# qurAI-amsterdam/SuperResolution_aniso_MRI

Hardware: AMD Instinct MI355X
Metric: training slices/sec (ae_combined, 160x160, latent=128) (higher is better)
Workload: dtype f32; 1 GPU; ACDC synthetic 12x(3x1x160x160) triplets, ae_combined latent=128 depth=32 scales=2, MSE synthesis loss (BASELINE configs[1]); global_batch_triplets=12, parallelism=dp1, init=reference Initializer, seed 892372, random weights, launch=captured HIP graph replay

## Files before the change

superresolution_aniso_mri_amd/csrc/aesr_kernels.h:

```cpp
#pragma once
#include "aesr_common.h"

struct IgemmArgs {
    const float* in; const float* wpk; const float* bias; const float* ysave; float* out;
    int N, H, W, Cin, CinP, Cout, CoutP, Ho, Wo, pad;
    int TI, TH, TW, tiles_y, tiles_x, nitems, dbg;
    int unused_;
    int ksplit;
    float* dbgbuf;
    int act, mask_act;
    float slope;
};
int aesr_launch_conv_igemm(const IgemmArgs& a, int KS, int NB, int MBW, hipStream_t st);
int aesr_launch_conv_ksplit_fixup(const float* partial, const float* bias, const float* ysave, float* out, size_t nelem, int Cout,
                                  int ksplit, int act, int mask_act, float slope, hipStream_t st);
int aesr_launch_pack_weights(const float* w, float* p, int Cout, int Cin, int KS, int KinP, int NoutP, int TN, int transpose, hipStream_t st);

struct WinoArgs {
    const float* in; const float* upk; const float* bias; const float* ysave; float* out;
    int N, H, W, Cin, CinP, Cout, CoutP;
    int TI, THt, TWt;
    int regs_y, regs_x, nitems;
    unsigned m_ncot, m_regs_x, m_regs_y;
    int act, mask_act;
    float slope;
    float* dbgbuf;
    int flags;
    int in_up2;
    int out_sum2;
    int bpi, nblk;
    unsigned m_bpi;
    int nw, rowP, imgP, patch_fl, sw_a, sw_m, sw_b;
    int xcd_map;
    double plan_cost;
    int nfull, tail_k;
    int ksplit, kchunks, split_bytes;
    unsigned m_ksplit;
    float* ws;
    size_t ws_floats;
    const float* post_scale; const float* post_shift;
    int post_pool;
};
int aesr_launch_conv_wino(const WinoArgs& a, hipStream_t st);
bool aesr_wino_res_ok(const WinoArgs& a);
int aesr_launch_conv_wino_res(const WinoArgs& a, hipStream_t st);
int aesr_wino_ring_mode();
bool aesr_wino_ring_takes(const WinoArgs& a);
int aesr_launch_conv_wino_ring(const WinoArgs& a, hipStream_t st);
size_t aesr_wino_ring_workspace_floats(const WinoArgs& a);
unsigned aesr_wino_ring_timeouts();
size_t aesr_wino_lds_bytes(int patch_pixels);

#define PACK_MAX_JOBS 32
struct PackJob { const float* w; float* p; int Cout, Cin, KS, KinP, NoutP, TN, transpose, block0; };
struct PackTable { int njobs, nblocks; PackJob job[PACK_MAX_JOBS]; };
int aesr_launch_pack_many(const PackTable& t, hipStream_t st);
enum { PREP_PACK = 0, PREP_WINO_PACK = 1, PREP_STEM_FOLD = 2, PREP_COUT1_FLIP = 3 };
struct PrepJob { const float* w; const float* aux0; const float* aux1; float* out; int kind, Cout, Cin, KS, KinP, NoutP, TN, transpose, block0; };
struct PrepTable { int njobs, nblocks; PrepJob job[PACK_MAX_JOBS]; };
int aesr_launch_prep_many(const PrepTable& t, hipStream_t st);
int aesr_launch_wino_pack_many(const PackTable& t, hipStream_t st);

struct WgradArgs {
    const float* x; const float* dy; float* slab;
    int N, H, W, Cin, CinP, Cout, CoutP, Ho, Wo, pad;
    int TH, TW, tiles_y, tiles_x, ntiles;
    int S;
    int PWS, TWS, PSX, PSD;
// ... 206 lines not shown
```

superresolution_aniso_mri_amd/csrc/conv_wgrad_wino.hip:

```cpp
#include <stdio.h>
#include <stdlib.h>

#include <type_traits>
#include <utility>

#include "aesr_kernels.h"

constexpr int WW_OOB = 0x70000000;
typedef float f32x2 __attribute__((ext_vector_type(2)));

template <int... I, class F>
__device__ __forceinline__ void ww_for(std::integer_sequence<int, I...>, F&& f) {
    (f(std::integral_constant<int, I>{}), ...);
}
template <int N, class F>
__device__ __forceinline__ void ww_rep(F&& f) { ww_for(std::make_integer_sequence<int, N>{}, f); }

__device__ __forceinline__ void ww_dma(__amdgpu_buffer_rsrc_t rs, float* lds_wave_base, int byte_off) {
    __builtin_amdgcn_raw_ptr_buffer_load_lds(rs, (__attribute__((address_space(3))) void*)lds_wave_base, 16, byte_off, 0, 0, 0);
}

#define WW_PK(dst, a, b, mods)                                                          \
    do {                                                                                \
        f32x2& d_ = dst;                                                                \
        const f32x2 a_ = a, b_ = b;                                                     \
        asm volatile("v_pk_add_f32 %0, %1, %2 " mods : "=v"(d_) : "v"(a_), "v"(b_));    \
    } while (0)
#define WW_M_ADD ""
#define WW_M_SUB "neg_lo:[0,1] neg_hi:[0,1]"
#define WW_M_T01 "op_sel:[0,0] op_sel_hi:[1,0] neg_lo:[0,1] neg_hi:[0,0]"
#define WW_M_T23 "op_sel:[1,0] op_sel_hi:[1,1] neg_lo:[1,0] neg_hi:[0,1]"
#define WW_M_LL "op_sel:[0,0] op_sel_hi:[0,0] neg_lo:[0,0] neg_hi:[0,1]"
#define WW_M_HH "op_sel:[1,1] op_sel_hi:[1,1] neg_lo:[0,0] neg_hi:[0,1]"
#define WW_M_SELF "op_sel:[0,1] op_sel_hi:[0,1] neg_lo:[0,0] neg_hi:[0,1]"

__device__ __forceinline__ f32x4 ww_sub4(f32x4 a, f32x4 b) {
    f32x2 lo, hi;
    const f32x2 alo = a.xy, ahi = a.zw, blo = b.xy, bhi = b.zw;
    asm("v_pk_add_f32 %0, %1, %2 " WW_M_SUB : "=v"(lo) : "v"(alo), "v"(blo));
    asm("v_pk_add_f32 %0, %1, %2 " WW_M_SUB : "=v"(hi) : "v"(ahi), "v"(bhi));
    return (f32x4){lo.x, lo.y, hi.x, hi.y};
}
typedef float f32x4u __attribute__((ext_vector_type(4), aligned(4)));

struct WwTile {
    int n, ty, tx;
};

constexpr int WW_NTS = 10;
constexpr int WW_DBG_WAVES = 4096 * 4;
template <int TH, int TW, bool STAMP, bool LEAN>
__global__ __launch_bounds__(256, 1) void conv_wgrad_wino_f32(WgradArgs a) {
    constexpr int CIT = 32, COT = 32;
    static_assert((TH == 16 && TW == 8) || (TH == 8 && TW == 16), "tiles: 8 k-steps, rows of whole 8-pixel DMA segments");
    constexpr int PH = TH + 2, PWL = TW == 8 ? 16 : 32, TWL = TW;
    constexpr int XFL = PH * PWL * 32, DFL = TH * TWL * 32;
    constexpr int KPR = TW >> 3;
    constexpr int SPR = PWL / 8, SPRD = TW / 8;
    constexpr int NXS = PH * SPR / 4, NDS = TH * SPRD / 4;
    constexpr int RXS = 4 / SPR, RDS = 4 / SPRD;
    static_assert(2 * (XFL + DFL) * 4 <= 160 * 1024 && (PH * SPR) % 4 == 0 && (TH * SPRD) % 4 == 0, "LDS / segment split");

    extern __shared__ __attribute__((aligned(16))) float lds[];
    unsigned long long ts[WW_NTS] = {};
#define WW_TS(k)                                          \
    if constexpr (STAMP) {                                \
        __builtin_amdgcn_sched_barrier(0);                \
        ts[k] = __builtin_amdgcn_s_memrealtime();         \
        __builtin_amdgcn_sched_barrier(0);                \
    }
    WW_TS(0)
    const int tid = threadIdx.x, lane = tid & 63;
    const int wave = __builtin_amdgcn_readfirstlane(tid >> 6);
    const int l15 = lane & 15, g = lane >> 4;
    const int nci = a.CinP / CIT, nchunks = nci * (a.CoutP / COT);
    int chunk, split;
// ... 100 lines not shown
                         : "=&v"(p0_), "=&v"(p1_) : "v"(ad), "n"(0), "n"(PWL / 2), "n"(PWL), "n"(3 * PWL / 2) : "memory");
        });
        ww_rep<4>([&](auto Kc) {
            constexpr int o = decltype(Kc)::value >> 1, e = decltype(Kc)::value & 1;
            const unsigned ad = ld[o][e] + (unsigned)(du * 4);
            f32x2& y_ = Mp[nb][o][e];
            asm volatile("ds_read2st64_b32 %0, %1 offset0:0 offset1:%2" : "=&v"(y_) : "v"(ad), "n"(TWL / 2) : "memory");
        });
    };
    auto op_transform = [&](int nb) {
        asm volatile("s_waitcnt lgkmcnt(0)" ::: "memory");
        ww_rep<2>([&](auto Ic) {
            constexpr int i = decltype(Ic)::value;
            f32x2 T[2][4];
            ww_rep<4>([&](auto Cc) {
                constexpr int c = decltype(Cc)::value;
                WW_PK(T[0][c], P[i][c][0], P[i][c][1], WW_M_T01);
                WW_PK(T[1][c], P[i][c][0], P[i][c][1], WW_M_T23);
            });
            ww_rep<2>([&](auto Sc) {
                constexpr int s_ = decltype(Sc)::value;
                WW_PK(Vp[nb][i][s_][0], T[s_][0], T[s_][2], WW_M_SUB);
                WW_PK(Vp[nb][i][s_][1], T[s_][1], T[s_][2], WW_M_ADD);
                WW_PK(Vp[nb][i][s_][2], T[s_][2], T[s_][1], WW_M_SUB);
                WW_PK(Vp[nb][i][s_][3], T[s_][1], T[s_][3], WW_M_SUB);
            });
        });
        ww_rep<2>([&](auto Oc) {
            constexpr int o = decltype(Oc)::value;
            WW_PK(Mp[nb][o][2], Mp[nb][o][0], Mp[nb][o][0], WW_M_SELF);
            WW_PK(Mp[nb][o][3], Mp[nb][o][1], Mp[nb][o][1], WW_M_SELF);
            WW_PK(Mp[nb][o][4], Mp[nb][o][0], Mp[nb][o][1], WW_M_LL);
            WW_PK(Mp[nb][o][7], Mp[nb][o][0], Mp[nb][o][1], WW_M_HH);
            WW_PK(Mp[nb][o][5], Mp[nb][o][2], Mp[nb][o][3], WW_M_LL);
            WW_PK(Mp[nb][o][6], Mp[nb][o][2], Mp[nb][o][3], WW_M_HH);
            accb[o] += Mp[nb][o][5][0];
        });
    };
    auto mfmas = [&](auto Q0c, auto Nc, int cb) {
        ww_rep<decltype(Nc)::value>([&](auto Dc) {
            constexpr int q = decltype(Q0c)::value + decltype(Dc)::value, x = q >> 2, i = (q >> 1) & 1, o = q & 1;
            constexpr int r = x >> 2, k = x & 3;
            constexpr int mi = k == 0 ? (r == 0 || r == 3 ? 0 : 2) : k == 3 ? (r == 0 || r == 3 ? 1 : 3) : 4 + r;
            constexpr int mh = k == 0 || k == 3 ? (r >= 2 ? 1 : 0) : k - 1;
            f32x4& acc_ = acc[x][i][o];
            const float va_ = Vp[cb][i][r >> 1][k][r & 1], vb_ = Mp[cb][o][mi][mh];
            asm volatile("v_mfma_f32_16x16x4_f32 %0, %1, %2, %0" : "+a"(acc_) : "v"(va_), "v"(vb_));
        });
    };
    auto step_xu = [&](int j, int buf) { const int ks = wave + 4 * j, tyl = ks / KPR, kx = ks - tyl * KPR; return buf * XFL + ((2 * tyl) * PWL + 8 * kx) * 32; };
    auto step_du = [&](int j, int buf) { const int ks = wave + 4 * j, tyl = ks / KPR, kx = ks - tyl * KPR; return buf * DFL + ((2 * tyl) * TWL + 8 * kx) * 32; };
    using C0 = std::integral_constant<int, 0>;
    using C16 = std::integral_constant<int, 16>;
    using C32 = std::integral_constant<int, 32>;

    long long tph[3] = {0, 0, 0}, tq = 0;
#define WW_STAMP(k)                                                   \
    if constexpr (STAMP) {                                            \
        const long long t_ = (long long)__builtin_amdgcn_s_memtime(); \
        tph[k] += t_ - tq;                                            \
        tq = t_;                                                      \
    }
    if constexpr (STAMP) tq = (long long)__builtin_amdgcn_s_memtime();

    WwTile t0, t1, t2;
    {
        t0.n = split / tpi;
        const int rem = split - t0.n * tpi;
        t0.ty = rem / a.tiles_x;
        t0.tx = rem - t0.ty * a.tiles_x;
        if (split >= a.ntiles) t0.n = a.N;
    }
    t1 = advance(t0);
    t2 = advance(t1);
    fetch(t0, 0);
    fetch(t1, 1);
    WW_TS(1)
    if constexpr (LEAN) {
        __builtin_amdgcn_sched_barrier(0);
        ww_rep<64>([&](auto Qc) {
            constexpr int q = decltype(Qc)::value;
            f32x4& acc_ = acc[q >> 2][(q >> 1) & 1][q & 1];
            acc_ = (f32x4){0.f, 0.f, 0.f, 0.f};
            asm volatile("" : "+a"(acc_));
        });
        __builtin_amdgcn_sched_barrier(0);
        if (8 * sgx < TW + 2) asm volatile("s_waitcnt vmcnt(%0)" ::"n"(NXS + NDS) : "memory");
        else asm volatile("s_waitcnt vmcnt(%0)" ::"n"(NDS) : "memory");
        __builtin_amdgcn_s_barrier();
    } else {
        asm volatile("s_waitcnt vmcnt(0)" ::: "memory");
        __syncthreads();
    }
    WW_TS(2)
    int buf = 0;
    op_read(step_xu(0, 0), step_du(0, 0), 0);
    op_transform(0);
    WW_STAMP(2)
    WW_TS(3)
    if (t0.n < a.N) do {
        __builtin_amdgcn_sched_barrier(0);
        op_read(step_xu(1, buf), step_du(1, buf), 1);
        mfmas(C0{}, C16{}, 0);
        op_transform(1);
        mfmas(C16{}, std::integral_constant<int, 48>{}, 0);
        __builtin_amdgcn_sched_barrier(0);
        WW_STAMP(0)
        asm volatile("s_waitcnt vmcnt(0) lgkmcnt(0)" ::: "memory");
        __syncthreads();
        WW_STAMP(1)
        __builtin_amdgcn_sched_barrier(0);
        op_read(step_xu(0, buf ^ 1), step_du(0, buf ^ 1), 0);
        mfmas(C0{}, C16{}, 1);
        __builtin_amdgcn_sched_barrier(0);
        fetch(t2, buf);
        __builtin_amdgcn_sched_barrier(0);
        mfmas(C16{}, C16{}, 1);
        op_transform(0);
        mfmas(C32{}, C32{}, 1);
        __builtin_amdgcn_sched_barrier(0);
        t0 = t1;
        t1 = t2;
        t2 = advance(t2);
        buf ^= 1;
    } while (t0.n < a.N);
    WW_STAMP(0)
    WW_TS(4)
    asm volatile("s_waitcnt vmcnt(0) lgkmcnt(0)" ::: "memory");
    __syncthreads();
    WW_TS(5)
    if (STAMP && lane == 0)
        for (int k = 0; k < 3; ++k) a.dbgbuf[(blockIdx.x * 4 + wave) * 3 + k] = (float)tph[k];

    if constexpr (!LEAN) {
        f32x4 dg[9][2][2];
#pragma unroll
        for (int i = 0; i < 2; ++i)
#pragma unroll
            for (int o = 0; o < 2; ++o) {
                f32x4 R[3][4];
#pragma unroll
                for (int j = 0; j < 4; ++j) {
                    const f32x4 u0_ = acc[0 + j][i][o], u1 = acc[4 + j][i][o], u2 = acc[8 + j][i][o], u3 = -acc[12 + j][i][o];
                    const f32x4 s = j == 3 ? (f32x4){-1.f, -1.f, -1.f, -1.f} : (f32x4){1.f, 1.f, 1.f, 1.f};
                    R[0][j] = s * (u0_ + 0.5f * (u1 + u2));
                    R[1][j] = s * (0.5f * (u1 - u2));
                    R[2][j] = s * (0.5f * (u1 + u2) + u3);
                }
#pragma unroll
                for (int r = 0; r < 3; ++r) {
                    dg[r * 3 + 0][i][o] = R[r][0] + 0.5f * (R[r][1] + R[r][2]);
                    dg[r * 3 + 1][i][o] = 0.5f * (R[r][1] - R[r][2]);
                    dg[r * 3 + 2][i][o] = 0.5f * (R[r][1] + R[r][2]) + R[r][3];
                }
            }
#pragma unroll
        for (int o = 0; o < 2; ++o) {
            accb[o] += __shfl_xor(accb[o], 16, 64);
            accb[o] += __shfl_xor(accb[o], 32, 64);
        }
        WW_TS(6)
        f32x4* ex = (f32x4*)lds;
        float* exb = lds + 4 * 36 * 64 * 4;
#pragma unroll
        for (int t = 0; t < 9; ++t)
#pragma unroll
// ... 21 lines not shown
                const int ci = ci0 + i * 16 + g * 4 + e;
                sl[t * plane + (size_t)ci * a.CoutP + co] = v[e];
            }
        }
        if (wave == 0 && do_bias && g == 0) {
#pragma unroll
            for (int o = 0; o < 2; ++o) {
                float bsum = exb[0 * 32 + o * 16 + l15];
#pragma unroll
                for (int w = 1; w < 4; ++w) bsum += exb[w * 32 + o * 16 + l15];
                sl[9 * plane + co0 + o * 16 + l15] = bsum;
            }
        }
    } else {
        const int ln = (int)__builtin_amdgcn_mbcnt_hi(~0u, __builtin_amdgcn_mbcnt_lo(~0u, 0u));
        const int e15 = ln & 15, eg = ln >> 4;
        float* const exf = lds;
        float* const exb = lds + 4 * 36 * 64 * 4;
        ww_rep<4>([&](auto Pc) {
            constexpr int i = decltype(Pc)::value >> 1, o = decltype(Pc)::value & 1;
            f32x4 R[3][4];
            ww_rep<4>([&](auto Jc) {
                constexpr int j = decltype(Jc)::value;
                const f32x4 u0_ = acc[0 + j][i][o], u1 = acc[4 + j][i][o], u2 = acc[8 + j][i][o], u3n = acc[12 + j][i][o];
                const f32x4 h = 0.5f * (u1 + u2);
                R[0][j] = u0_ + h;
                R[1][j] = 0.5f * ww_sub4(u1, u2);
                R[2][j] = ww_sub4(h, u3n);
            });
            ww_rep<3>([&](auto Rc) {
                constexpr int r = decltype(Rc)::value;
                const f32x4 h = 0.5f * (R[r][1] + R[r][2]);
                const f32x4 d[3] = {R[r][0] + h, 0.5f * ww_sub4(R[r][1], R[r][2]), ww_sub4(h, R[r][3])};
                ww_rep<3>([&](auto Cc) {
                    constexpr int c = decltype(Cc)::value, blk = (r * 3 + c) * 4 + i * 2 + o;
                    float* const p = exf + (wave * 36 + blk) * 256 + ln;
#pragma unroll
                    for (int e = 0; e < 4; ++e) p[e * 64] = d[c][e];
                });
            });
        });
#pragma unroll
        for (int o = 0; o < 2; ++o) {
            accb[o] += __shfl_xor(accb[o], 16, 64);
            accb[o] += __shfl_xor(accb[o], 32, 64);
        }
        if (eg == 0) {
// ... 28 lines not shown
            }
        }
    }
    if constexpr (STAMP) {
        WW_TS(8)
        asm volatile("s_waitcnt vmcnt(0)" ::: "memory");
        WW_TS(9)
        if (lane == 0) {
            unsigned long long* out = (unsigned long long*)(a.dbgbuf + WW_DBG_WAVES * 3) + (size_t)(blockIdx.x * 4 + wave) * WW_NTS;
            for (int k = 0; k < WW_NTS; ++k) out[k] = ts[k];
        }
    }
}

size_t aesr_wgrad_wino_lds_bytes(int TH, int TW) {
    const size_t xfl = (size_t)(TH + 2) * (TW == 8 ? 16 : 32) * 32, dfl = (size_t)TH * TW * 32;
    const size_t bufs = 2 * (xfl + dfl) * sizeof(float);
    const size_t exch = ((size_t)4 * 36 * 64 * 4 + 4 * 32) * sizeof(float);
    return bufs > exch ? bufs : exch;
}

bool aesr_wgrad_wino_tile_ok(int TH, int TW) { return (TH == 16 && TW == 8) || (TH == 8 && TW == 16); }

template <int TH, int TW, bool LEAN>
static int launch_wgrad_wino(const WgradArgs& a, hipStream_t st) {
    const size_t shmem = aesr_wgrad_wino_lds_bytes(TH, TW);
    static bool attr_set[AESR_MAX_DEVICES] = {}, attr_set_dbg[AESR_MAX_DEVICES] = {};
    if (int e = aesr_lds_opt_in((const void*)conv_wgrad_wino_f32<TH, TW, false, LEAN>, "conv_wgrad_wino_f32", attr_set)) return e;
    (void)aesr_lds_opt_in((const void*)conv_wgrad_wino_f32<TH, TW, true, LEAN>, "conv_wgrad_wino_f32", attr_set_dbg);
    dim3 grid(a.S * (a.CinP / 32) * (a.CoutP / 32));
    if (getenv("AESR_WGRAD_WINO_DBG") && grid.x * 4 <= (unsigned)WW_DBG_WAVES) {
        constexpr size_t dbytes = (size_t)WW_DBG_WAVES * (3 * sizeof(float) + WW_NTS * sizeof(unsigned long long));
        static float* dbuf = nullptr;
        if (!dbuf) (void)hipMalloc(&dbuf, dbytes);
        WgradArgs b = a;
        b.dbgbuf = dbuf;
        hipLaunchKernelGGL((conv_wgrad_wino_f32<TH, TW, true, LEAN>), grid, dim3(256), shmem, st, b);
        (void)hipStreamSynchronize(st);
        static float host[dbytes / sizeof(float)];
        (void)hipMemcpy(host, dbuf, dbytes, hipMemcpyDeviceToHost);
        const unsigned nw = grid.x * 4;
        double s3[3] = {0, 0, 0};
        for (unsigned i = 0; i < nw; ++i) for (int k = 0; k < 3; ++k) s3[k] += host[i * 3 + k];
        const double visits = (double)((a.ntiles + a.S - 1) / a.S);
        const int nks = (TH >> 1) * (TW >> 3);
        fprintf(stderr, "[wgrad-wino stamps] grid=%u tile %dx%d S=%d lean=%d (%.0f visits, %d k-steps = %d MFMA cycles per wave and visit) per visit, cycles: "
                "k-step loop %.0f | barrier %.0f || fill %.0f\n", grid.x, TH, TW, a.S, (int)LEAN, visits, nks, nks / 4 * 64 * 32,
                s3[0] / grid.x / 4 / visits, s3[1] / grid.x / 4 / visits, s3[2] / grid.x / 4);
        const unsigned long long* ts = (const unsigned long long*)(host + WW_DBG_WAVES * 3);
        unsigned long long first = ~0ull, last = 0;
        for (unsigned i = 0; i < nw; ++i) {
            if (ts[(size_t)i * WW_NTS] < first) first = ts[(size_t)i * WW_NTS];
            if (ts[(size_t)i * WW_NTS + WW_NTS - 1] > last) last = ts[(size_t)i * WW_NTS + WW_NTS - 1];
        }
        double ph[WW_NTS] = {}, skew = 0, skew_max = 0;
        for (unsigned i = 0; i < nw; ++i) {
            const unsigned long long* t = ts + (size_t)i * WW_NTS;
            const double e = (double)(t[0] - first) * 0.01;
            skew += e;
            if (e > skew_max) skew_max = e;
            for (int k = 1; k < WW_NTS; ++k) ph[k] += (double)(t[k] - t[k - 1]) * 0.01;
        }
        for (int k = 1; k < WW_NTS; ++k) ph[k] /= nw;
        fprintf(stderr, "[wgrad-wino life] %d->%d N=%d %dx%d lean=%d: span %.2f us | per wave, us: entry behind first wave %.2f (max %.2f) | DMA issue %.2f | "
                "tile wait+barrier %.2f | first operands %.2f | loop %.2f (%.2f per visit) | drain wait+barrier %.2f | dg %.2f | exchange+barrier %.2f | "
                "slab stores issued %.2f | stores retired %.2f || outside the loop %.2f\n", a.Cin, a.Cout, a.N, a.H, a.W, (int)LEAN,
                (double)(last - first) * 0.01, skew / nw, skew_max, ph[1], ph[2], ph[3], ph[4], ph[4] / visits, ph[5], ph[6], ph[7], ph[8], ph[9],
                ph[1] + ph[2] + ph[3] + ph[5] + ph[6] + ph[7] + ph[8] + ph[9]);
        return AESR_OK;
    }
    hipLaunchKernelGGL((conv_wgrad_wino_f32<TH, TW, false, LEAN>), grid, dim3(256), shmem, st, a);
    AESR_LAUNCH_CHECK("conv_wgrad_wino_f32");
    return AESR_OK;
}

int aesr_launch_conv_wgrad_wino(const WgradArgs& a, hipStream_t st) {
    if ((size_t)a.H * a.W * a.Cin * 4 >= (size_t)0x10000000 || (size_t)a.H * a.W * a.Cout * 4 >= (size_t)0x10000000) {
        aesr_set_error("conv_wgrad_wino: images of 256 MB or more need 64-bit lane offsets (not built)");
        return AESR_ERR_UNSUPPORTED;
    }
    if (a.x_up2 && ((a.H | a.W) & 1)) {
        aesr_set_error("conv_wgrad_wino: the folded Upsample(x2) needs even convolution sizes (got %dx%d)", a.H, a.W);
        return AESR_ERR_ARG;
    }
    if (!aesr_wgrad_wino_tile_ok(a.TH, a.TW) || a.pad != 1 || a.Ho != a.H || a.Wo != a.W) {
        aesr_set_error("conv_wgrad_wino: tile %dx%d is not 16x8 or 8x16 (or not 3x3 / padding 1)", a.TH, a.TW);
        return AESR_ERR_ARG;
    }
    if (a.CinP % 32 != 0 || a.CoutP % 32 != 0 || a.Cin != a.CinP || a.Cout != a.CoutP || a.S < 1 || a.S > a.ntiles ||
        a.tiles_y != ceil_div(a.H, a.TH) || a.tiles_x != ceil_div(a.W, a.TW) || a.ntiles != a.N * a.tiles_y * a.tiles_x) {
        aesr_set_error("conv_wgrad_wino: channel counts must be multiples of 32 and the tile grid consistent (S=%d, %d tiles)", a.S, a.ntiles);
        return AESR_ERR_ARG;
    }
    static const bool lean_env = [] { const char* e = getenv("AESR_WGRAD_WINO_LEAN"); return !(e && *e && atoi(e) == 0); }();
    const bool lean = lean_env && (size_t)a.CinP * a.CoutP * 40 < ((size_t)1 << 32);
    if (a.TH == 16) return lean ? launch_wgrad_wino<16, 8, true>(a, st) : launch_wgrad_wino<16, 8, false>(a, st);
    return lean ? launch_wgrad_wino<8, 16, true>(a, st) : launch_wgrad_wino<8, 16, false>(a, st);
}
```

superresolution_aniso_mri_amd/csrc/conv_wino_res.hip:

```cpp
#include <stdio.h>
#include <stdlib.h>

#include <type_traits>
#include <vector>

#include "aesr_kernels.h"
#include "conv_wino_tile.h"

constexpr int WR_NT = 512;
constexpr int WR_RP = 260;
constexpr int WR_PFL = 10 * WR_RP;

template <int WR_TN, bool MASK, bool POST = false, bool STAMP = false>
__global__ __launch_bounds__(WR_NT, 2) void conv_wino_res_f32(WinoArgs a) {
    constexpr int WR_NB = WR_TN / 16;
    constexpr int WR_WFL = 16 * 4 * WR_TN * 4;
    extern __shared__ __attribute__((aligned(16))) float lds[];
    const int tid = threadIdx.x, lane = tid & 63;
    const int wave = __builtin_amdgcn_readfirstlane(tid >> 6);
    unsigned long long stamp[14] = {};
    int stamped_items = 0;
#define WR_STAMP(k)                                                          \
    if constexpr (STAMP) {                                                   \
        if (stamped_items == 0) stamp[k] = __builtin_amdgcn_s_memrealtime(); \
    }
    WR_STAMP(0)
    const int l15 = lane & 15, g = lane >> 4;
    const int ncot = a.CoutP / WR_TN, nchunks = a.CinP >> 4;
    const bool xmap = a.xcd_map != 0;
    const int xcd = blockIdx.x & 7, lw = blockIdx.x >> 3;
    const int cot = xmap ? lw % ncot : blockIdx.x % ncot;
    const int wgc = xmap ? lw / ncot : blockIdx.x / ncot;
    const int nwgc = xmap ? (gridDim.x >> 3) / ncot : gridDim.x / ncot;
    const int co0 = cot * WR_TN;
    float* const ldsW = lds;
    float* const ldsP = lds + nchunks * WR_WFL + wave * WR_PFL;
    float* const ldsBias = lds + nchunks * WR_WFL + 8 * WR_PFL;

// ... 56 lines not shown
        fetch(item, 0);
    }
    WR_STAMP(1)
    if (tid < WR_TN) ldsBias[tid] = bias_v;
    asm volatile("s_waitcnt vmcnt(0)" ::: "memory");
    __syncthreads();
    WR_STAMP(2)

    f32x4 acc[16][WR_NB];
    int cc = 0;
    bool after_stores = false;
    while (item < a.nblk) {
        if (after_stores) asm volatile("s_waitcnt vmcnt(%0)" ::"n"(4 * WR_NB) : "memory");
        else asm volatile("s_waitcnt vmcnt(0)" ::: "memory");
        if constexpr (STAMP) {
            if (stamped_items == 0 && cc < 4) stamp[3 + 2 * cc] = __builtin_amdgcn_s_memrealtime();
        }
        f32x4 t[4][4];
#pragma unroll
        for (int i = 0; i < 4; ++i)
#pragma unroll
            for (int j = 0; j < 4; ++j) t[i][j] = *(const f32x4*)(ldsP + (j < 2 ? offA : offB) + i * WR_RP + j * 16);
        const float* wb = wbl + cc * WR_WFL;
        constexpr int PP = (WR_NB == 1) ? 2 : 1;
        f32x4 wnx[PP][WR_NB];
#pragma unroll
        for (int pp = 0; pp < PP; ++pp)
#pragma unroll
            for (int nb = 0; nb < WR_NB; ++nb) wnx[pp][nb] = *(const f32x4*)(wb + pp * (4 * WR_TN * 4) + nb * 64);
        asm volatile("s_waitcnt lgkmcnt(0)" ::: "memory");
        const int cur_n = in_n, cur_y0 = in_y0, cur_x0 = in_x0;
        const bool last = cc + 1 == nchunks;
        if (last) {
            slot += 8;
            item = item_of(slot);
            if (item < a.nblk) {
                locate(item);
                fetch(item, 0);
            }
        } else {
            fetch(item, cc + 1);
        }
        WINO_ROW_HALF(t)
        auto positions = [&](auto firstc) {
            constexpr bool FIRST = decltype(firstc)::value;
            f32x4 vnx[PP];
#pragma unroll
            for (int pp = 0; pp < PP; ++pp) vnx[pp] = WINO_V(t, pp >> 2, pp & 3);
#pragma unroll
            for (int grp = 0; grp < 16 / PP; ++grp) {
                f32x4 wc[PP][WR_NB], vc[PP];
#pragma unroll
                for (int pp = 0; pp < PP; ++pp) {
                    vc[pp] = vnx[pp];
#pragma unroll
                    for (int nb = 0; nb < WR_NB; ++nb) wc[pp][nb] = wnx[pp][nb];
                }
                if (grp + 1 < 16 / PP) {
#pragma unroll
                    for (int pp = 0; pp < PP; ++pp) {
                        const int xn = (grp + 1) * PP + pp;
#pragma unroll
                        for (int nb = 0; nb < WR_NB; ++nb) wnx[pp][nb] = *(const f32x4*)(wb + xn * (4 * WR_TN * 4) + nb * 64);
                        vnx[pp] = WINO_V(t, xn >> 2, xn & 3);
                    }
                }
                __builtin_amdgcn_sched_barrier(0);
#pragma unroll
                for (int r = 0; r < 4; ++r)
#pragma unroll
                    for (int pp = 0; pp < PP; ++pp)
#pragma unroll
                        for (int nb = 0; nb < WR_NB; ++nb) {
                            const int xi = grp * PP + pp;
                            f32x4 c = acc[xi][nb];
                            if (FIRST && r == 0) c = xi == 5 ? *(const f32x4*)(ldsBias + nb * 16 + 4 * g) : (f32x4){0.f, 0.f, 0.f, 0.f};
                            acc[xi][nb] = __builtin_amdgcn_mfma_f32_16x16x4f32(wc[pp][nb][r], vc[pp][r], c, 0, 0, 0);
                        }
                __builtin_amdgcn_sched_barrier(0);
            }
        };
        if (cc == 0) positions(std::true_type{});
        else positions(std::false_type{});
        if constexpr (STAMP) {
            if (stamped_items == 0 && cc < 4) stamp[4 + 2 * cc] = __builtin_amdgcn_s_memrealtime();
        }
        after_stores = false;
        if (!last) {
            ++cc;
            continue;
        }
        cc = 0;
        {
            const int y0 = cur_y0 + 2 * ty, x0 = cur_x0 + 2 * tx;
            WINO_STORE_TILE(WR_NB, MASK, POST, true, cur_n, y0, x0, co0, g, 0)
        }
        after_stores = !MASK && !halfout;
        WR_STAMP(11)
        if constexpr (STAMP) ++stamped_items;
    }
    asm volatile("s_waitcnt vmcnt(0)" ::: "memory");
    if constexpr (STAMP) {
        stamp[12] = __builtin_amdgcn_s_memrealtime();
        stamp[13] = (unsigned long long)stamped_items;
        if (lane == 0) {
            unsigned long long* dst = (unsigned long long*)a.dbgbuf + ((size_t)blockIdx.x * 8 + wave) * 16;
#pragma unroll
            for (int k = 0; k < 14; ++k) dst[k] = stamp[k];
        }
    }
#undef WR_STAMP
}

static int wino_res_tn(const WinoArgs& a) {
    if (a.CinP > 32) return 16;
    static const int forced = getenv("AESR_WINO_RES_TN") ? atoi(getenv("AESR_WINO_RES_TN")) : 0;
    if (forced == 16 || forced == 32) return forced;
    const long nblk = (long)a.N * ceil_div(a.H, 8) * ceil_div(a.W, 8);
// ... 59 lines not shown
            "entry behind first wave %.2f (max %.2f) | DMA issue %.2f | prologue wait+barrier %.2f |", b.Cin, b.Cout, b.N, b.H, b.W, WR_TN, grid, busy,
            grid * 8, items, (double)(t_last - t_first) * 0.01, sum[0] * q, ramp_max * 0.01, sum[1] * q, sum[2] * q);
    for (int c = 0; c < nch; ++c) fprintf(stderr, " chunk %d: wait %.2f work %.2f |", c, sum[3 + 2 * c] * q, sum[4 + 2 * c] * q);
    fprintf(stderr, " epilogue %.2f | rest of the wave %.2f\n", sum[11] * q, sum[12] * q);
    double ex[8] = {}, ex_min[8], ex_max[8] = {};
    int nw[8] = {};
    for (int w = 0; w < 8; ++w) ex_min[w] = 1e30;
    for (size_t w = 0; w < (size_t)grid * 8; ++w) {
        const unsigned long long* s_ = &host[w * 16];
        if (!s_[13]) continue;
        const double e = (double)(s_[12] - t_first) * 0.01;
        const int k = (int)(w & 7);
        ex[k] += e; ++nw[k];
        if (e < ex_min[k]) ex_min[k] = e;
        if (e > ex_max[k]) ex_max[k] = e;
    }
    fprintf(stderr, "[wino-res stamps] exit of wave w behind the grid's first entry, us (mean [min .. max] over the workgroups):");
    for (int w = 0; w < 8; ++w)
        if (nw[w]) fprintf(stderr, "  w%d %.1f [%.1f .. %.1f]", w, ex[w] / nw[w], ex_min[w], ex_max[w]);
    fprintf(stderr, "\n");
    return AESR_OK;
}

template <int WR_TN, bool MASK, bool POST = false>
static int wino_res_launch_one(const WinoArgs& a, hipStream_t st) {
    const size_t shmem = wino_res_lds_bytes(a.CinP, WR_TN);
    static bool attr_set[AESR_MAX_DEVICES] = {};
    if (int e = aesr_lds_opt_in((const void*)conv_wino_res_f32<WR_TN, MASK, POST>, "conv_wino_res_f32", attr_set)) return e;
    const int ncot = a.CoutP / WR_TN;
    int grid = 256 / ncot * ncot;
    if (const char* e = getenv("AESR_WINO_GRID")) grid = atoi(e) / ncot * ncot;
    static const int wpw = getenv("AESR_WINO_RES_WPW") ? atoi(getenv("AESR_WINO_RES_WPW")) : 4;
    const int per_cot = ceil_div(a.nblk, wpw >= 1 && wpw <= 8 ? wpw : 4);
    if (grid / ncot > per_cot) grid = per_cot * ncot;
    if (grid < ncot) grid = ncot;
    WinoArgs b = a;
    static const int xmap_on = getenv("AESR_WINO_XCD") ? atoi(getenv("AESR_WINO_XCD")) : 1;
    b.xcd_map = (xmap_on && grid % (8 * ncot) == 0 && a.nblk >= 8 * (grid / ncot)) ? 1 : 0;
    if constexpr (!MASK && !POST) {
        if (getenv("AESR_WINO_RES_DBG")) return wino_res_stamped<WR_TN>(b, grid, shmem, st);
    }
    hipLaunchKernelGGL((conv_wino_res_f32<WR_TN, MASK, POST>), dim3(grid), dim3(WR_NT), shmem, st, b);
    AESR_LAUNCH_CHECK("conv_wino_res_f32");
    return AESR_OK;
}

int aesr_launch_conv_wino_res(const WinoArgs& a_in, hipStream_t st) {
    WinoArgs a = a_in;
    a.TI = 1; a.THt = 4; a.TWt = 4;
    a.regs_y = ceil_div(a.H, 8);
    a.regs_x = ceil_div(a.W, 8);
    a.bpi = a.regs_y * a.regs_x;
    a.nblk = a.N * a.bpi;
    const int TN = wino_res_tn(a);
    a.nitems = a.nblk * (a.CoutP / TN);
    a.m_bpi = aesr_magic_u32(a.bpi); a.m_regs_x = aesr_magic_u32(a.regs_x);
    if (((unsigned long long)a.nblk + 4096) * (unsigned)(a.bpi + a.regs_x) >= ((unsigned long long)1 << 31) || (size_t)a.H * a.W * a.Cin * 4 >= (size_t)0x10000000) {
        aesr_set_error("conv_wino_res: %d blocks exceed the exact range of the item decomposition (or images of 256 MB and more)", a.nblk);
        return AESR_ERR_UNSUPPORTED;
    }
    if (wino_res_lds_bytes(a.CinP, TN) > (size_t)160 * 1024) {
        aesr_set_error("conv_wino_res: %d input channels do not fit the resident filter", a.CinP);
        return AESR_ERR_ARG;
    }
    if (a.post_scale) {
        if (a.ysave || a.out_sum2 || !a.post_shift) {
            aesr_set_error("conv_wino_res: the folded eval-mode BatchNorm is a forward epilogue (no derivative mask, no 2x2-summing output)");
            return AESR_ERR_ARG;
        }
        return TN == 32 ? wino_res_launch_one<32, false, true>(a, st) : wino_res_launch_one<16, false, true>(a, st);
    }
    if (TN == 32) return a.ysave ? wino_res_launch_one<32, true>(a, st) : wino_res_launch_one<32, false>(a, st);
    return a.ysave ? wino_res_launch_one<16, true>(a, st) : wino_res_launch_one<16, false>(a, st);
}
```

superresolution_aniso_mri_amd/csrc/conv_wino_tile.h:

```cpp
#pragma once
#include "aesr_common.h"

constexpr int WINO_OOB = 0x70000000;

__device__ __forceinline__ void wino_dma(__amdgpu_buffer_rsrc_t rs, float* lds_wave_base, int byte_off, int uniform_off = 0) {
    __builtin_amdgcn_raw_ptr_buffer_load_lds(rs, (__attribute__((address_space(3))) void*)lds_wave_base, 16, byte_off, uniform_off, 0, 0);
}
__device__ __forceinline__ f32x4 wino_ld(__amdgpu_buffer_rsrc_t rs, int byte_off) {
    return __builtin_bit_cast(f32x4, __builtin_amdgcn_raw_buffer_load_b128(rs, byte_off, 0, 0));
}
__device__ __forceinline__ void wino_st(__amdgpu_buffer_rsrc_t rs, int byte_off, f32x4 v) {
    __builtin_amdgcn_raw_buffer_store_b128(__builtin_bit_cast(__attribute__((__vector_size__(4 * sizeof(unsigned int)))) unsigned int, v), rs, byte_off, 0, 0);
}

#define WINO_DIV(x, m) ((m) ? (int)__umulhi((unsigned)(x), (m)) : (int)(x))

__device__ __forceinline__ float wino_slope(int act, float slope) { return act == ACT_LRELU ? slope : (act == ACT_RELU ? 0.f : 1.f); }

#define WINO_ROW_HALF(t)                                                            \
    _Pragma("unroll") for (int j_ = 0; j_ < 4; ++j_) {                              \
        const f32x4 d0_ = t[0][j_], d1_ = t[1][j_], d2_ = t[2][j_], d3_ = t[3][j_]; \
        t[0][j_] = aesr_sub4(d0_, d2_);                                             \
        t[1][j_] = d1_ + d2_;                                                       \
        t[2][j_] = aesr_sub4(d2_, d1_);                                             \
// ... 47 lines not shown
                        _Pragma("unroll") for (int e = 0; e < 4; ++e) o[e] = 1.f / (1.f + expf(-o[e]));                                      \
                    }                                                                                                                        \
                    if (MASK) {                                                                                                              \
                        _Pragma("unroll") for (int e = 0; e < 4; ++e) o[e] *= (ys[p][q][e] > 0.f ? 1.f : mslope);                            \
                    }                                                                                                                        \
                    if (POST) {                                                                                                              \
                        if (a.post_pool) prow = q == 0 ? o : prow + o;                                                                       \
                        else wino_st(rs_out, ob[p][q] + cob, o * psc + psh);                         \
                    } else {                                                                                                                 \
                        wino_st(rs_out, ob[p][q] + cob + (so), o);                                                                           \
                    }                                                                                                                        \
                }                                                                                                                            \
                if ((POST) && a.post_pool) pm = p == 0 ? prow : pm + prow;                                                                   \
            }                                                                                                                                \
            if ((POST) && a.post_pool) {                                                                                                     \
                     \
                                                                        \
                const f32x4 m = pm * 0.25f;                                                          \
                const int obs = ((okn) && (y0) + 1 < a.H && (x0) + 1 < a.W) ? (((n) * outH + ((y0) >> 1)) * outW + ((x0) >> 1)) * a.Cout * 4 : WINO_OOB; \
                wino_st(rs_out, obs + cob, m * psc + psh);                                                                                   \
            }                                                                                                                                \
        }                                                                                                                                    \
    }
```

Baseline: 16320 slices/s.

## Skip structurally zero Winograd positions for 2x-upsampled convolutions

For convolutions whose input is nearest-upsampled by 2 (or whose data gradient sums 2x2 outputs), the Winograd F(2,3) transform has repeated rows and columns, so 7 of the 16 transform positions are redundant. The forward/dgrad residency kernel and the weight-gradient kernel gain a NINE template variant that runs MFMAs for only 9 positions, skips the dead transform ops, and uses a dedicated output transform. It is enabled by default via an environment flag. It relies on the algebraic identity holding exactly and adds more kernel instantiations.

```diff
diff --git a/superresolution_aniso_mri_amd/csrc/aesr_kernels.h b/superresolution_aniso_mri_amd/csrc/aesr_kernels.h
--- a/superresolution_aniso_mri_amd/csrc/aesr_kernels.h
+++ b/superresolution_aniso_mri_amd/csrc/aesr_kernels.h
@@ -44,6 +44,7 @@
 int aesr_launch_conv_wino(const WinoArgs& a, hipStream_t st);
 bool aesr_wino_res_ok(const WinoArgs& a);
 int aesr_launch_conv_wino_res(const WinoArgs& a, hipStream_t st);
+bool aesr_wino_up2_nine();
 int aesr_wino_ring_mode();
 bool aesr_wino_ring_takes(const WinoArgs& a);
 int aesr_launch_conv_wino_ring(const WinoArgs& a, hipStream_t st);
diff --git a/superresolution_aniso_mri_amd/csrc/conv_wgrad_wino.hip b/superresolution_aniso_mri_amd/csrc/conv_wgrad_wino.hip
--- a/superresolution_aniso_mri_amd/csrc/conv_wgrad_wino.hip
+++ b/superresolution_aniso_mri_amd/csrc/conv_wgrad_wino.hip
@@ -41,6 +41,7 @@
     asm("v_pk_add_f32 %0, %1, %2 " WW_M_SUB : "=v"(hi) : "v"(ahi), "v"(bhi));
     return (f32x4){lo.x, lo.y, hi.x, hi.y};
 }
+#define WW_Z4 ((f32x4){0.f, 0.f, 0.f, 0.f})
 typedef float f32x4u __attribute__((ext_vector_type(4), aligned(4)));
 
 struct WwTile {
@@ -49,9 +50,15 @@
 
 constexpr int WW_NTS = 10;
 constexpr int WW_DBG_WAVES = 4096 * 4;
-template <int TH, int TW, bool STAMP, bool LEAN>
+template <bool NINE>
+__host__ __device__ constexpr int ww_xi(int k) { return NINE ? 4 * (k / 3 == 2 ? 3 : k / 3) + (k % 3 == 2 ? 3 : k % 3) : k; }
+template <bool NINE>
+__host__ __device__ constexpr bool ww_dead(int x) { return NINE && ((x >> 2) == 2 || (x & 3) == 2); }
+
+template <int TH, int TW, bool STAMP, bool LEAN, bool NINE = false>
 __global__ __launch_bounds__(256, 1) void conv_wgrad_wino_f32(WgradArgs a) {
     constexpr int CIT = 32, COT = 32;
+    constexpr int NPOS = NINE ? 9 : 16, NQ = 4 * NPOS;
     static_assert((TH == 16 && TW == 8) || (TH == 8 && TW == 16), "tiles: 8 k-steps, rows of whole 8-pixel DMA segments");
     constexpr int PH = TH + 2, PWL = TW == 8 ? 16 : 32, TWL = TW;
     constexpr int XFL = PH * PWL * 32, DFL = TH * TWL * 32;
@@ -198,7 +205,7 @@
                 constexpr int s_ = decltype(Sc)::value;
                 WW_PK(Vp[nb][i][s_][0], T[s_][0], T[s_][2], WW_M_SUB);
                 WW_PK(Vp[nb][i][s_][1], T[s_][1], T[s_][2], WW_M_ADD);
-                WW_PK(Vp[nb][i][s_][2], T[s_][2], T[s_][1], WW_M_SUB);
+                if constexpr (!NINE) WW_PK(Vp[nb][i][s_][2], T[s_][2], T[s_][1], WW_M_SUB);
                 WW_PK(Vp[nb][i][s_][3], T[s_][1], T[s_][3], WW_M_SUB);
             });
         });
@@ -209,13 +216,13 @@
             WW_PK(Mp[nb][o][4], Mp[nb][o][0], Mp[nb][o][1], WW_M_LL);
             WW_PK(Mp[nb][o][7], Mp[nb][o][0], Mp[nb][o][1], WW_M_HH);
             WW_PK(Mp[nb][o][5], Mp[nb][o][2], Mp[nb][o][3], WW_M_LL);
-            WW_PK(Mp[nb][o][6], Mp[nb][o][2], Mp[nb][o][3], WW_M_HH);
+            if constexpr (!NINE) WW_PK(Mp[nb][o][6], Mp[nb][o][2], Mp[nb][o][3], WW_M_HH);
             accb[o] += Mp[nb][o][5][0];
         });
     };
     auto mfmas = [&](auto Q0c, auto Nc, int cb) {
         ww_rep<decltype(Nc)::value>([&](auto Dc) {
-            constexpr int q = decltype(Q0c)::value + decltype(Dc)::value, x = q >> 2, i = (q >> 1) & 1, o = q & 1;
+            constexpr int q = decltype(Q0c)::value + decltype(Dc)::value, x = ww_xi<NINE>(q >> 2), i = (q >> 1) & 1, o = q & 1;
             constexpr int r = x >> 2, k = x & 3;
             constexpr int mi = k == 0 ? (r == 0 || r == 3 ? 0 : 2) : k == 3 ? (r == 0 || r == 3 ? 1 : 3) : 4 + r;
             constexpr int mh = k == 0 || k == 3 ? (r >= 2 ? 1 : 0) : k - 1;
@@ -227,8 +234,8 @@
     auto step_xu = [&](int j, int buf) { const int ks = wave + 4 * j, tyl = ks / KPR, kx = ks - tyl * KPR; return buf * XFL + ((2 * tyl) * PWL + 8 * kx) * 32; };
     auto step_du = [&](int j, int buf) { const int ks = wave + 4 * j, tyl = ks / KPR, kx = ks - tyl * KPR; return buf * DFL + ((2 * tyl) * TWL + 8 * kx) * 32; };
     using C0 = std::integral_constant<int, 0>;
-    using C16 = std::integral_constant<int, 16>;
-    using C32 = std::integral_constant<int, 32>;
+    using Q1 = std::integral_constant<int, NQ / 4>;
+    using Q2 = std::integral_constant<int, NQ / 2>;
 
     long long tph[3] = {0, 0, 0}, tq = 0;
 #define WW_STAMP(k)                                                   \
@@ -254,9 +261,9 @@
     WW_TS(1)
     if constexpr (LEAN) {
         __builtin_amdgcn_sched_barrier(0);
-        ww_rep<64>([&](auto Qc) {
+        ww_rep<NQ>([&](auto Qc) {
             constexpr int q = decltype(Qc)::value;
-            f32x4& acc_ = acc[q >> 2][(q >> 1) & 1][q & 1];
+            f32x4& acc_ = acc[ww_xi<NINE>(q >> 2)][(q >> 1) & 1][q & 1];
             acc_ = (f32x4){0.f, 0.f, 0.f, 0.f};
             asm volatile("" : "+a"(acc_));
         });
@@ -277,9 +284,9 @@
     if (t0.n < a.N) do {
         __builtin_amdgcn_sched_barrier(0);
         op_read(step_xu(1, buf), step_du(1, buf), 1);
-        mfmas(C0{}, C16{}, 0);
+        mfmas(C0{}, Q1{}, 0);
         op_transform(1);
-        mfmas(C16{}, std::integral_constant<int, 48>{}, 0);
+        mfmas(Q1{}, std::integral_constant<int, NQ - NQ / 4>{}, 0);
         __builtin_amdgcn_sched_barrier(0);
         WW_STAMP(0)
         asm volatile("s_waitcnt vmcnt(0) lgkmcnt(0)" ::: "memory");
@@ -287,13 +294,13 @@
         WW_STAMP(1)
         __builtin_amdgcn_sched_barrier(0);
         op_read(step_xu(0, buf ^ 1), step_du(0, buf ^ 1), 0);
-        mfmas(C0{}, C16{}, 1);
+        mfmas(C0{}, Q1{}, 1);
         __builtin_amdgcn_sched_barrier(0);
         fetch(t2, buf);
         __builtin_amdgcn_sched_barrier(0);
-        mfmas(C16{}, C16{}, 1);
+        mfmas(Q1{}, Q1{}, 1);
         op_transform(0);
-        mfmas(C32{}, C32{}, 1);
+        mfmas(Q2{}, Q2{}, 1);
         __builtin_amdgcn_sched_barrier(0);
         t0 = t1;
         t1 = t2;
@@ -317,7 +324,8 @@
                 f32x4 R[3][4];
 #pragma unroll
                 for (int j = 0; j < 4; ++j) {
-                    const f32x4 u0_ = acc[0 + j][i][o], u1 = acc[4 + j][i][o], u2 = acc[8 + j][i][o], u3 = -acc[12 + j][i][o];
+                    const f32x4 u0_ = ww_dead<NINE>(0 + j) ? WW_Z4 : acc[0 + j][i][o], u1 = ww_dead<NINE>(4 + j) ? WW_Z4 : acc[4 + j][i][o];
+                    const f32x4 u2 = ww_dead<NINE>(8 + j) ? WW_Z4 : acc[8 + j][i][o], u3 = -(ww_dead<NINE>(12 + j) ? WW_Z4 : acc[12 + j][i][o]);
                     const f32x4 s = j == 3 ? (f32x4){-1.f, -1.f, -1.f, -1.f} : (f32x4){1.f, 1.f, 1.f, 1.f};
                     R[0][j] = s * (u0_ + 0.5f * (u1 + u2));
                     R[1][j] = s * (0.5f * (u1 - u2));
@@ -385,7 +393,8 @@
             f32x4 R[3][4];
             ww_rep<4>([&](auto Jc) {
                 constexpr int j = decltype(Jc)::value;
-                const f32x4 u0_ = acc[0 + j][i][o], u1 = acc[4 + j][i][o], u2 = acc[8 + j][i][o], u3n = acc[12 + j][i][o];
+                const f32x4 u0_ = ww_dead<NINE>(0 + j) ? WW_Z4 : acc[0 + j][i][o], u1 = ww_dead<NINE>(4 + j) ? WW_Z4 : acc[4 + j][i][o];
+                const f32x4 u2 = ww_dead<NINE>(8 + j) ? WW_Z4 : acc[8 + j][i][o], u3n = ww_dead<NINE>(12 + j) ? WW_Z4 : acc[12 + j][i][o];
                 const f32x4 h = 0.5f * (u1 + u2);
                 R[0][j] = u0_ + h;
                 R[1][j] = 0.5f * ww_sub4(u1, u2);
@@ -460,12 +469,12 @@
 
 bool aesr_wgrad_wino_tile_ok(int TH, int TW) { return (TH == 16 && TW == 8) || (TH == 8 && TW == 16); }
 
-template <int TH, int TW, bool LEAN>
+template <int TH, int TW, bool LEAN, bool NINE = false>
 static int launch_wgrad_wino(const WgradArgs& a, hipStream_t st) {
     const size_t shmem = aesr_wgrad_wino_lds_bytes(TH, TW);
     static bool attr_set[AESR_MAX_DEVICES] = {}, attr_set_dbg[AESR_MAX_DEVICES] = {};
-    if (int e = aesr_lds_opt_in((const void*)conv_wgrad_wino_f32<TH, TW, false, LEAN>, "conv_wgrad_wino_f32", attr_set)) return e;
-    (void)aesr_lds_opt_in((const void*)conv_wgrad_wino_f32<TH, TW, true, LEAN>, "conv_wgrad_wino_f32", attr_set_dbg);
+    if (int e = aesr_lds_opt_in((const void*)conv_wgrad_wino_f32<TH, TW, false, LEAN, NINE>, "conv_wgrad_wino_f32", attr_set)) return e;
+    (void)aesr_lds_opt_in((const void*)conv_wgrad_wino_f32<TH, TW, true, LEAN, NINE>, "conv_wgrad_wino_f32", attr_set_dbg);
     dim3 grid(a.S * (a.CinP / 32) * (a.CoutP / 32));
     if (getenv("AESR_WGRAD_WINO_DBG") && grid.x * 4 <= (unsigned)WW_DBG_WAVES) {
         constexpr size_t dbytes = (size_t)WW_DBG_WAVES * (3 * sizeof(float) + WW_NTS * sizeof(unsigned long long));
@@ -473,7 +482,7 @@
         if (!dbuf) (void)hipMalloc(&dbuf, dbytes);
         WgradArgs b = a;
         b.dbgbuf = dbuf;
-        hipLaunchKernelGGL((conv_wgrad_wino_f32<TH, TW, true, LEAN>), grid, dim3(256), shmem, st, b);
+        hipLaunchKernelGGL((conv_wgrad_wino_f32<TH, TW, true, LEAN, NINE>), grid, dim3(256), shmem, st, b);
         (void)hipStreamSynchronize(st);
         static float host[dbytes / sizeof(float)];
         (void)hipMemcpy(host, dbuf, dbytes, hipMemcpyDeviceToHost);
@@ -483,7 +492,7 @@
         const double visits = (double)((a.ntiles + a.S - 1) / a.S);
         const int nks = (TH >> 1) * (TW >> 3);
         fprintf(stderr, "[wgrad-wino stamps] grid=%u tile %dx%d S=%d lean=%d (%.0f visits, %d k-steps = %d MFMA cycles per wave and visit) per visit, cycles: "
-                "k-step loop %.0f | barrier %.0f || fill %.0f\n", grid.x, TH, TW, a.S, (int)LEAN, visits, nks, nks / 4 * 64 * 32,
+                "k-step loop %.0f | barrier %.0f || fill %.0f\n", grid.x, TH, TW, a.S, (int)LEAN, visits, nks, nks / 4 * (NINE ? 36 : 64) * 32,
                 s3[0] / grid.x / 4 / visits, s3[1] / grid.x / 4 / visits, s3[2] / grid.x / 4);
         const unsigned long long* ts = (const unsigned long long*)(host + WW_DBG_WAVES * 3);
         unsigned long long first = ~0ull, last = 0;
@@ -507,7 +516,7 @@
                 ph[1] + ph[2] + ph[3] + ph[5] + ph[6] + ph[7] + ph[8] + ph[9]);
         return AESR_OK;
     }
-    hipLaunchKernelGGL((conv_wgrad_wino_f32<TH, TW, false, LEAN>), grid, dim3(256), shmem, st, a);
+    hipLaunchKernelGGL((conv_wgrad_wino_f32<TH, TW, false, LEAN, NINE>), grid, dim3(256), shmem, st, a);
     AESR_LAUNCH_CHECK("conv_wgrad_wino_f32");
     return AESR_OK;
 }
@@ -532,6 +541,10 @@
     }
     static const bool lean_env = [] { const char* e = getenv("AESR_WGRAD_WINO_LEAN"); return !(e && *e && atoi(e) == 0); }();
     const bool lean = lean_env && (size_t)a.CinP * a.CoutP * 40 < ((size_t)1 << 32);
-    if (a.TH == 16) return lean ? launch_wgrad_wino<16, 8, true>(a, st) : launch_wgrad_wino<16, 8, false>(a, st);
-    return lean ? launch_wgrad_wino<8, 16, true>(a, st) : launch_wgrad_wino<8, 16, false>(a, st);
-}
+    if (!(a.x_up2 && aesr_wino_up2_nine())) {
+        if (a.TH == 16) return lean ? launch_wgrad_wino<16, 8, true>(a, st) : launch_wgrad_wino<16, 8, false>(a, st);
+        return lean ? launch_wgrad_wino<8, 16, true>(a, st) : launch_wgrad_wino<8, 16, false>(a, st);
+    }
+    if (a.TH == 16) return lean ? launch_wgrad_wino<16, 8, true, true>(a, st) : launch_wgrad_wino<16, 8, false, true>(a, st);
+    return lean ? launch_wgrad_wino<8, 16, true, true>(a, st) : launch_wgrad_wino<8, 16, false, true>(a, st);
+}
diff --git a/superresolution_aniso_mri_amd/csrc/conv_wino_res.hip b/superresolution_aniso_mri_amd/csrc/conv_wino_res.hip
--- a/superresolution_aniso_mri_amd/csrc/conv_wino_res.hip
+++ b/superresolution_aniso_mri_amd/csrc/conv_wino_res.hip
@@ -11,9 +11,14 @@
 constexpr int WR_RP = 260;
 constexpr int WR_PFL = 10 * WR_RP;
 
-template <int WR_TN, bool MASK, bool POST = false, bool STAMP = false>
+template <bool NINE>
+__host__ __device__ constexpr int wr_xi(int k) { return NINE ? 4 * (k / 3 == 2 ? 3 : k / 3) + (k % 3 == 2 ? 3 : k % 3) : k; }
+
+template <int WR_TN, bool MASK, bool POST = false, bool STAMP = false, bool NINE = false>
 __global__ __launch_bounds__(WR_NT, 2) void conv_wino_res_f32(WinoArgs a) {
+    static_assert(!NINE || (!MASK && !POST && !STAMP), "the nine-position form: plain forward / 2x2-summing data gradient only");
     constexpr int WR_NB = WR_TN / 16;
+    constexpr int NPOS = NINE ? 9 : 16;
     constexpr int WR_WFL = 16 * 4 * WR_TN * 4;
     extern __shared__ __attribute__((aligned(16))) float lds[];
     const int tid = threadIdx.x, lane = tid & 63;
@@ -116,12 +121,12 @@
 #pragma unroll
             for (int j = 0; j < 4; ++j) t[i][j] = *(const f32x4*)(ldsP + (j < 2 ? offA : offB) + i * WR_RP + j * 16);
         const float* wb = wbl + cc * WR_WFL;
-        constexpr int PP = (WR_NB == 1) ? 2 : 1;
+        constexpr int PP = (WR_NB == 1) ? (NINE ? 3 : 2) : 1;
         f32x4 wnx[PP][WR_NB];
 #pragma unroll
         for (int pp = 0; pp < PP; ++pp)
 #pragma unroll
-            for (int nb = 0; nb < WR_NB; ++nb) wnx[pp][nb] = *(const f32x4*)(wb + pp * (4 * WR_TN * 4) + nb * 64);
+            for (int nb = 0; nb < WR_NB; ++nb) wnx[pp][nb] = *(const f32x4*)(wb + wr_xi<NINE>(pp) * (4 * WR_TN * 4) + nb * 64);
         asm volatile("s_waitcnt lgkmcnt(0)" ::: "memory");
         const int cur_n = in_n, cur_y0 = in_y0, cur_x0 = in_x0;
         const bool last = cc + 1 == nchunks;
@@ -140,9 +145,9 @@
             constexpr bool FIRST = decltype(firstc)::value;
             f32x4 vnx[PP];
 #pragma unroll
-            for (int pp = 0; pp < PP; ++pp) vnx[pp] = WINO_V(t, pp >> 2, pp & 3);
-#pragma unroll
-            for (int grp = 0; grp < 16 / PP; ++grp) {
+            for (int pp = 0; pp < PP; ++pp) vnx[pp] = WINO_V(t, wr_xi<NINE>(pp) >> 2, wr_xi<NINE>(pp) & 3);
+#pragma unroll
+            for (int grp = 0; grp < NPOS / PP; ++grp) {
                 f32x4 wc[PP][WR_NB], vc[PP];
 #pragma unroll
                 for (int pp = 0; pp < PP; ++pp) {
@@ -150,10 +155,10 @@
 #pragma unroll
                     for (int nb = 0; nb < WR_NB; ++nb) wc[pp][nb] = wnx[pp][nb];
                 }
-                if (grp + 1 < 16 / PP) {
+                if (grp + 1 < NPOS / PP) {
 #pragma unroll
                     for (int pp = 0; pp < PP; ++pp) {
-                        const int xn = (grp + 1) * PP + pp;
+                        const int xn = wr_xi<NINE>((grp + 1) * PP + pp);
 #pragma unroll
                         for (int nb = 0; nb < WR_NB; ++nb) wnx[pp][nb] = *(const f32x4*)(wb + xn * (4 * WR_TN * 4) + nb * 64);
                         vnx[pp] = WINO_V(t, xn >> 2, xn & 3);
@@ -166,7 +171,7 @@
                     for (int pp = 0; pp < PP; ++pp)
 #pragma unroll
                         for (int nb = 0; nb < WR_NB; ++nb) {
-                            const int xi = grp * PP + pp;
+                            const int xi = wr_xi<NINE>(grp * PP + pp);
                             f32x4 c = acc[xi][nb];
                             if (FIRST && r == 0) c = xi == 5 ? *(const f32x4*)(ldsBias + nb * 16 + 4 * g) : (f32x4){0.f, 0.f, 0.f, 0.f};
                             acc[xi][nb] = __builtin_amdgcn_mfma_f32_16x16x4f32(wc[pp][nb][r], vc[pp][r], c, 0, 0, 0);
@@ -187,7 +192,11 @@
         cc = 0;
         {
             const int y0 = cur_y0 + 2 * ty, x0 = cur_x0 + 2 * tx;
-            WINO_STORE_TILE(WR_NB, MASK, POST, true, cur_n, y0, x0, co0, g, 0)
+            if constexpr (NINE) {
+                WINO_STORE_TILE9(WR_NB, true, cur_n, y0, x0, co0, g, 0)
+            } else {
+                WINO_STORE_TILE(WR_NB, MASK, POST, true, cur_n, y0, x0, co0, g, 0)
+            }
         }
         after_stores = !MASK && !halfout;
         WR_STAMP(11)
@@ -293,11 +302,11 @@
     return AESR_OK;
 }
 
-template <int WR_TN, bool MASK, bool POST = false>
+template <int WR_TN, bool MASK, bool POST = false, bool NINE = false>
 static int wino_res_launch_one(const WinoArgs& a, hipStream_t st) {
     const size_t shmem = wino_res_lds_bytes(a.CinP, WR_TN);
     static bool attr_set[AESR_MAX_DEVICES] = {};
-    if (int e = aesr_lds_opt_in((const void*)conv_wino_res_f32<WR_TN, MASK, POST>, "conv_wino_res_f32", attr_set)) return e;
+    if (int e = aesr_lds_opt_in((const void*)conv_wino_res_f32<WR_TN, MASK, POST, false, NINE>, "conv_wino_res_f32", attr_set)) return e;
     const int ncot = a.CoutP / WR_TN;
     int grid = 256 / ncot * ncot;
     if (const char* e = getenv("AESR_WINO_GRID")) grid = atoi(e) / ncot * ncot;
@@ -308,12 +317,17 @@
     WinoArgs b = a;
     static const int xmap_on = getenv("AESR_WINO_XCD") ? atoi(getenv("AESR_WINO_XCD")) : 1;
     b.xcd_map = (xmap_on && grid % (8 * ncot) == 0 && a.nblk >= 8 * (grid / ncot)) ? 1 : 0;
-    if constexpr (!MASK && !POST) {
+    if constexpr (!MASK && !POST && !NINE) {
         if (getenv("AESR_WINO_RES_DBG")) return wino_res_stamped<WR_TN>(b, grid, shmem, st);
     }
-    hipLaunchKernelGGL((conv_wino_res_f32<WR_TN, MASK, POST>), dim3(grid), dim3(WR_NT), shmem, st, b);
+    hipLaunchKernelGGL((conv_wino_res_f32<WR_TN, MASK, POST, false, NINE>), dim3(grid), dim3(WR_NT), shmem, st, b);
     AESR_LAUNCH_CHECK("conv_wino_res_f32");
     return AESR_OK;
+}
+
+bool aesr_wino_up2_nine() {
+    static const bool on = [] { const char* e = getenv("AESR_WINO_UP2_NINE"); return !(e && *e && atoi(e) == 0); }();
+    return on;
 }
 
 int aesr_launch_conv_wino_res(const WinoArgs& a_in, hipStream_t st) {
@@ -341,6 +355,9 @@
         }
         return TN == 32 ? wino_res_launch_one<32, false, true>(a, st) : wino_res_launch_one<16, false, true>(a, st);
     }
-    if (TN == 32) return a.ysave ? wino_res_launch_one<32, true>(a, st) : wino_res_launch_one<32, false>(a, st);
-    return a.ysave ? wino_res_launch_one<16, true>(a, st) : wino_res_launch_one<16, false>(a, st);
-}
+    if (!((a.in_up2 || a.out_sum2) && !a.ysave && aesr_wino_up2_nine())) {
+        if (TN == 32) return a.ysave ? wino_res_launch_one<32, true>(a, st) : wino_res_launch_one<32, false>(a, st);
+        return a.ysave ? wino_res_launch_one<16, true>(a, st) : wino_res_launch_one<16, false>(a, st);
+    }
+    return TN == 32 ? wino_res_launch_one<32, false, false, true>(a, st) : wino_res_launch_one<16, false, false, true>(a, st);
+}
diff --git a/superresolution_aniso_mri_amd/csrc/conv_wino_tile.h b/superresolution_aniso_mri_amd/csrc/conv_wino_tile.h
--- a/superresolution_aniso_mri_amd/csrc/conv_wino_tile.h
+++ b/superresolution_aniso_mri_amd/csrc/conv_wino_tile.h
@@ -93,3 +93,44 @@
             }                                                                                                                                \
         }                                                                                                                                    \
     }
+
+#define WINO_STORE_TILE9(NB, okn, n, y0, x0, co0, g, so)                                                                                     \
+    {                                                                                                                                        \
+        int ob[2][2];                                                                                                                        \
+        _Pragma("unroll") for (int p = 0; p < 2; ++p)                                                                                        \
+            _Pragma("unroll") for (int q = 0; q < 2; ++q)                                                                                    \
+                ob[p][q] = ((okn) && (y0) + p < a.H && (x0) + q < a.W) ? (((n) * a.H + (y0) + p) * a.W + (x0) + q) * a.Cout * 4 : WINO_OOB; \
+        _Pragma("unroll") for (int nb = 0; nb < (NB); ++nb) {                                                                                \
+            const int co = (co0) + nb * 16 + 4 * (g);                                                                                        \
+            const int cob = co < a.Cout ? co * 4 : WINO_OOB;                                                                                 \
+            if (a.out_sum2) {                                                                                                                \
+                const f32x4 Q0 = aesr_sub4(acc[0][nb] + 2.f * acc[4][nb], acc[12][nb]);                                                      \
+                const f32x4 Q1 = aesr_sub4(acc[1][nb] + 2.f * acc[5][nb], acc[13][nb]);                                                      \
+                const f32x4 Q3 = aesr_sub4(acc[3][nb] + 2.f * acc[7][nb], acc[15][nb]);                                                      \
+                const f32x4 s = aesr_sub4(Q0 + 2.f * Q1, Q3);                                                                                \
+                const int obs = ((okn) && (y0) < a.H && (x0) < a.W) ? (((n) * outH + ((y0) >> 1)) * outW + ((x0) >> 1)) * a.Cout * 4 : WINO_OOB; \
+                wino_st(rs_out, obs + cob + (so), s);                                                                                        \
+                continue;                                                                                                                    \
+            }                                                                                                                                \
+            f32x4 P[2][4];                                                                                                                   \
+            _Pragma("unroll") for (int j = 0; j < 4; ++j) {                                                                                  \
+                if (j == 2) continue;                                                                                                        \
+                P[0][j] = acc[0 + j][nb] + acc[4 + j][nb];                                                                                   \
+                P[1][j] = aesr_sub4(acc[4 + j][nb], acc[12 + j][nb]);                                                                        \
+            }                                                                                                                                \
+            _Pragma("unroll") for (int p = 0; p < 2; ++p) {                                                                                  \
+                f32x4 Y[2];                                                                                                                  \
+                Y[0] = P[p][0] + P[p][1];                                                                                                    \
+                Y[1] = aesr_sub4(P[p][1], P[p][3]);                                                                                          \
+                _Pragma("unroll") for (int q = 0; q < 2; ++q) {                                                                              \
+                    f32x4 o = Y[q];                                                                                                          \
+                    const f32x4 os = o * nslope;                                                                                             \
+                    _Pragma("unroll") for (int e = 0; e < 4; ++e) o[e] = fmaxf(o[e], os[e]);                                                 \
+                    if (sigm) {                                                                                                              \
+                        _Pragma("unroll") for (int e = 0; e < 4; ++e) o[e] = 1.f / (1.f + expf(-o[e]));                                      \
+                    }                                                                                                                        \
+                    wino_st(rs_out, ob[p][q] + cob + (so), o);                                                                               \
+                }                                                                                                                            \
+            }                                                                                                                                \
+        }                                                                                                                                    \
+    }
```

Measured after the change: 17160 slices/s, median of 6. 5.2% higher.
